# skyepurchase/MeatModeler

Hardware: AMD Instinct MI355X
Metric: descriptor-match pairs/sec + BA residuals/sec, 500×1080p frames, 1/2/4/8 GPU (higher is better)
Workload: dtype u8/int32 (match), f64 (BA); 1 GPU; 500 frames 1920x1080, 4000 ORB kpts/frame, BF Hamming 2-NN + ratio, track linking, 2-view DLT, full BA (TRF, Schur, f64 MFMA Cholesky); frames=500, height=1080, width=1920, nfeatures=4000, parallelism=pairs/points x1

## Files before the change

### meatmodeler_amd/csrc/ba.hip

```cpp
#include "ba_eval.h"


namespace {

template <bool FIXED>
__device__ __forceinline__ const double *cam_at(const double *__restrict__ cams, const double *__restrict__ fxc, int F, int f) {
    if constexpr (FIXED)
        return f < F ? cams + (size_t)f * 6 : fxc + (size_t)(f - F) * 6;
    else
        return cams + (size_t)f * 6;
}

template <bool FIXED>
__device__ __forceinline__ void ba_residual_body(mm_ba_problem pb, const double *__restrict__ cams, const double *__restrict__ fxc,
                                                          const double *__restrict__ pts, const CamCoef *__restrict__ ctab, double *__restrict__ res,
                                                          double *__restrict__ partial, const unsigned bx, const unsigned gx) {
    __shared__ double sm[4];
    __shared__ double Ks[9];
    if (threadIdx.x < 9) Ks[threadIdx.x] = pb.K[threadIdx.x];
    __syncthreads();
    double acc = 0;
    for (int64_t o = (int64_t)bx * 256 + threadIdx.x; o < pb.O; o += (int64_t)gx * 256) {
        Proj pr;
        const int f = pb.fi[o];
// ... 46 lines not shown
}
__global__ __launch_bounds__(256) void sum_partials_publish_kernel(const double *__restrict__ partial, int n,
                                                                   double *__restrict__ board, int cost_slot, int count,
                                                                   MMHostBoard *hb, unsigned long long seq) { sum_partials_publish_body(partial, n, board, cost_slot, count, hb, seq, blockIdx.x, gridDim.x); }

__global__ __launch_bounds__(256) void ba_jacobian_kernel(mm_ba_problem pb, const double *__restrict__ cams,
                                                          const double *__restrict__ pts, const CamCoef *__restrict__ ctab, double *__restrict__ Jc,
                                                          double *__restrict__ Jp) {
    __shared__ double Ks[9];
    if (threadIdx.x < 9) Ks[threadIdx.x] = pb.K[threadIdx.x];
    __syncthreads();
    int64_t o = (int64_t)blockIdx.x * 256 + threadIdx.x;
    if (o >= pb.O) return;
    Proj pr;
    const int f = pb.fi[o];
    ba_eval_cc<true, true>(cams + (size_t)f * 6, ctab[f],
                           pts + (size_t)pb.pi[o] * 3, Ks, pb.obs[2 * o], pb.obs[2 * o + 1], pr);
#pragma unroll
    for (int k = 0; k < 6; ++k) {
        Jc[o * 12 + k] = pr.Jc[0][k];
        Jc[o * 12 + 6 + k] = pr.Jc[1][k];
    }
#pragma unroll
    for (int k = 0; k < 3; ++k) {
        Jp[o * 6 + k] = pr.Jp[0][k];
        Jp[o * 6 + 3 + k] = pr.Jp[1][k];
    }
}

#ifndef MM_PB_LANES
#define MM_PB_LANES 4
#endif
constexpr int PB_LANES = MM_PB_LANES;
template <bool FIXED>
__device__ __forceinline__ void ba_point_blocks_body(mm_ba_problem pb, const double *__restrict__ cams, const double *__restrict__ fxc,
                                                              const double *__restrict__ pts, const CamCoef *__restrict__ ctab, double *__restrict__ C,
                                                              double *__restrict__ gp, const unsigned bx, const unsigned gx) {
    __shared__ double Ks[9];
    if (threadIdx.x < 9) Ks[threadIdx.x] = pb.K[threadIdx.x];
    __syncthreads();
    const int sub = threadIdx.x & (PB_LANES - 1);
    const int p = bx * (256 / PB_LANES) + (threadIdx.x / PB_LANES);
    const bool live = p < pb.P;
    double c[9] = {0, 0, 0, 0, 0, 0, 0, 0, 0};
    if (live) {
        const double *Xp = pts + (size_t)p * 3;
        const int e_end = pb.pt_ptr[p + 1];
        for (int e = pb.pt_ptr[p] + sub; e < e_end; e += PB_LANES) {
            const int o = pb.pt_obs[e];
            Proj pr;
            const int f = pb.fi[o];
            ba_eval_cc<false, true>(cam_at<FIXED>(cams, fxc, pb.F, f), ctab[f], Xp, Ks, pb.obs[2 * (size_t)o], pb.obs[2 * (size_t)o + 1], pr);
#pragma unroll
            for (int m = 0; m < 2; ++m) {
                const double j0 = pr.Jp[m][0], j1 = pr.Jp[m][1], j2 = pr.Jp[m][2];
                const double r = m == 0 ? pr.r0 : pr.r1;
                c[0] += j0 * j0; c[1] += j0 * j1; c[2] += j0 * j2;
                c[3] += j1 * j1; c[4] += j1 * j2; c[5] += j2 * j2;
                c[6] += j0 * r; c[7] += j1 * r; c[8] += j2 * r;
            }
        }
    }
#pragma unroll
    for (int off = 1; off < PB_LANES; off <<= 1) {
        double t[9];
#pragma unroll
        for (int q = 0; q < 9; ++q) t[q] = __shfl_xor(c[q], off, 64);
#pragma unroll
        for (int q = 0; q < 9; ++q) c[q] += t[q];
    }
    if (live && sub == 0) {
        double *Cp = C + (size_t)p * 6;
#pragma unroll
        for (int q = 0; q < 6; ++q) Cp[q] = c[q];
        gp[(size_t)p * 3] = c[6]; gp[(size_t)p * 3 + 1] = c[7]; gp[(size_t)p * 3 + 2] = c[8];
    }
}
__global__ __launch_bounds__(256) void ba_point_blocks_kernel(mm_ba_problem pb, const double *__restrict__ cams,
                                                              const double *__restrict__ pts, const CamCoef *__restrict__ ctab, double *__restrict__ C,
                                                              double *__restrict__ gp) { ba_point_blocks_body<false>(pb, cams, nullptr, pts, ctab, C, gp, blockIdx.x, gridDim.x); }
__global__ __launch_bounds__(256) void ba_point_blocks_fixed_kernel(mm_ba_problem pb, const double *__restrict__ cams, const double *__restrict__ fxc,
                                                                    const double *__restrict__ pts, const CamCoef *__restrict__ ctab, double *__restrict__ C,
// ... 29 lines not shown
            acc[21 + i] += pr.Jc[0][i] * pr.r0 + pr.Jc[1][i] * pr.r1;
        }
    }
    block_sum_n<27, 256>(acc, smn);
    if (threadIdx.x == 0) {
        int t = 0;
#pragma unroll
        for (int i = 0; i < 6; ++i) {
#pragma unroll
            for (int j = i; j < 6; ++j) {
                B[(size_t)f * 36 + i * 6 + j] = acc[t];
                B[(size_t)f * 36 + j * 6 + i] = acc[t];
                ++t;
            }
            gc[(size_t)f * 6 + i] = acc[21 + i];
        }
    }
}
__global__ __launch_bounds__(256) void ba_camera_blocks_kernel(mm_ba_problem pb, const double *__restrict__ cams,
                                                               const double *__restrict__ pts, double *__restrict__ B,
                                                               double *__restrict__ gc) { ba_camera_blocks_body(pb, cams, pts, B, gc, blockIdx.x, gridDim.x); }

__global__ __launch_bounds__(256) void ba_normal_eq_kernel(mm_ba_problem pb, const double *__restrict__ cams, const double *__restrict__ pts,
                                                           const CamCoef *__restrict__ ctab, double *__restrict__ B, double *__restrict__ gc,
                                                           double *__restrict__ C, double *__restrict__ gp) {
    if ((int)blockIdx.x < pb.F) ba_camera_blocks_body(pb, cams, pts, B, gc, blockIdx.x, (unsigned)pb.F);
    else ba_point_blocks_body<false>(pb, cams, nullptr, pts, ctab, C, gp, blockIdx.x - (unsigned)pb.F, gridDim.x - (unsigned)pb.F);
}
__global__ __launch_bounds__(256) void ba_normal_eq_fixed_kernel(mm_ba_problem pb, const double *__restrict__ cams, const double *__restrict__ fxc,
                                                                 const double *__restrict__ pts, const CamCoef *__restrict__ ctab, double *__restrict__ B,
                                                                 double *__restrict__ gc, double *__restrict__ C, double *__restrict__ gp) {
    if ((int)blockIdx.x < pb.F) ba_camera_blocks_body(pb, cams, pts, B, gc, blockIdx.x, (unsigned)pb.F);
    else ba_point_blocks_body<true>(pb, cams, fxc, pts, ctab, C, gp, blockIdx.x - (unsigned)pb.F, gridDim.x - (unsigned)pb.F);
}

__global__ __launch_bounds__(256) void ba_jvp_kernel(mm_ba_problem pb, const double *__restrict__ cams,
                                                     const double *__restrict__ pts, const CamCoef *__restrict__ ctab, const double *__restrict__ wc,
                                                     const double *__restrict__ wp, double *__restrict__ out) {
    __shared__ double Ks[9];
    if (threadIdx.x < 9) Ks[threadIdx.x] = pb.K[threadIdx.x];
    __syncthreads();
    int64_t o = (int64_t)blockIdx.x * 256 + threadIdx.x;
    if (o >= pb.O) return;
    const int f = pb.fi[o], p = pb.pi[o];
    Proj pr;
    ba_eval_cc<true, true>(cams + (size_t)f * 6, ctab[f],
                           pts + (size_t)p * 3, Ks, pb.obs[2 * o], pb.obs[2 * o + 1], pr);
    double y0 = 0, y1 = 0;
    if (wc) {
#pragma unroll
        for (int k = 0; k < 6; ++k) {
            double w = wc[(size_t)f * 6 + k];
            y0 += pr.Jc[0][k] * w;
            y1 += pr.Jc[1][k] * w;
        }
    }
    if (wp) {
#pragma unroll
        for (int k = 0; k < 3; ++k) {
            double w = wp[(size_t)p * 3 + k];
            y0 += pr.Jp[0][k] * w;
            y1 += pr.Jp[1][k] * w;
        }
    }
    out[2 * o] = y0;
    out[2 * o + 1] = y1;
// ... 127 lines not shown
                                                                double *__restrict__ dp, const unsigned bx, const unsigned gx) {
    const int sub = threadIdx.x & (PB_LANES - 1);
    const int p = bx * (256 / PB_LANES) + (threadIdx.x / PB_LANES);
    const bool live = p < pb.P;
    double t[3] = {0.0, 0.0, 0.0};
    if (live) {
        const int e_end = pb.pt_ptr[p + 1];
        for (int e = pb.pt_ptr[p] + sub; e < e_end; e += PB_LANES) {
            t[0] += T[3 * (size_t)e];
            t[1] += T[3 * (size_t)e + 1];
            t[2] += T[3 * (size_t)e + 2];
        }
    }
#pragma unroll
    for (int off = 1; off < PB_LANES; off <<= 1) {
        double u[3];
#pragma unroll
        for (int q = 0; q < 3; ++q) u[q] = __shfl_xor(t[q], off, 64);
#pragma unroll
        for (int q = 0; q < 3; ++q) t[q] += u[q];
    }
    if (live && sub == 0) {
        const double t0 = gp[(size_t)p * 3] - t[0], t1 = gp[(size_t)p * 3 + 1] - t[1], t2 = gp[(size_t)p * 3 + 2] - t[2];
        const double *c = Cinv + (size_t)p * 6;
        dp[(size_t)p * 3] = c[0] * t0 + c[1] * t1 + c[2] * t2;
        dp[(size_t)p * 3 + 1] = c[1] * t0 + c[3] * t1 + c[4] * t2;
        dp[(size_t)p * 3 + 2] = c[2] * t0 + c[4] * t1 + c[5] * t2;
    }
}
__global__ __launch_bounds__(256) void ba_backsub_points_kernel(mm_ba_problem pb, const double *__restrict__ T,
                                                                const double *__restrict__ Cinv, const double *__restrict__ gp,
                                                                double *__restrict__ dp) { ba_backsub_points_body(pb, T, Cinv, gp, dp, blockIdx.x, gridDim.x); }

__device__ __forceinline__ void cam_coef_body(const double *__restrict__ cams, int F, CamCoef *__restrict__ tab, const unsigned bx, const unsigned gx) {
    const int f = bx * 256 + threadIdx.x;
    if (f < F) tab[f] = cam_coef_of(cams + (size_t)f * 6);
}
__global__ __launch_bounds__(256) void cam_coef_kernel(const double *__restrict__ cams, int F, CamCoef *__restrict__ tab) { cam_coef_body(cams, F, tab, blockIdx.x, gridDim.x); }

int check_pb(mm_ctx *ctx, const mm_ba_problem *pb, const char *who) {
    if (!ctx) return MM_ERR_ARG;
    if (!pb || pb->F < 0 || pb->P < 0 || pb->O < 0 || !pb->K) return mm_fail(ctx, MM_ERR_ARG, "%s: bad problem", who);
    if (pb->O > 0 && (!pb->fi || !pb->pi || !pb->obs)) return mm_fail(ctx, MM_ERR_ARG, "%s: null observation arrays", who);
    return MM_OK;
}

constexpr int RES_BLOCKS = 2048;
constexpr int JVP_MAX_WG = 2048;
inline int res_wg_cap() {
    static const int cap = [] {
        const char *e = getenv("MM_RES_WG");
        const int v = e ? atoi(e) : RES_BLOCKS;
        return v < 1 ? 1 : (v > RES_BLOCKS ? RES_BLOCKS : v);
    }();
    return cap;
}
inline int jvp_wg_cap() {
    static const int cap = [] {
        const char *e = getenv("MM_JVP_WG");
        const int v = e ? atoi(e) : 1024;
        return v < 1 ? 1 : (v > JVP_MAX_WG ? JVP_MAX_WG : v);
    }();
    return cap;
}

__device__ __forceinline__ void trf_damping_body(const double *__restrict__ gh2, const double *__restrict__ d11, double Delta,
// ... 94 lines not shown
        ctx->cam_tab_for = cams;
        ctx->cam_tab_F = F;
    }
    if (ctx->fx_F > 0 && !ctx->fx_tab_ok) {
        MM_LAUNCH(ctx, "cam_coef_kernel", cam_coef_kernel, dim3((ctx->fx_F + 255) / 256), dim3(256), 0, ctx->fx_cams, ctx->fx_F,
                  (CamCoef *)ctx->cam_tab + F);
        ctx->fx_tab_ok = true;
    }
    *tab_out = ctx->cam_tab;
    return MM_OK;
}
int mm_cam_table_adopt(mm_ctx *ctx, const double *cams, int F, void **tab_out) {
    const int rows = F + ctx->fx_F;
    if (rows > ctx->cam_tab_cap) {
        if (ctx->cam_tab) (void)hipFree(ctx->cam_tab);
        ctx->cam_tab = nullptr;
        ctx->cam_tab_cap = 0;
        const int cap = rows < 1024 ? 1024 : rows + rows / 2;
        MM_HIP(ctx, hipMalloc(&ctx->cam_tab, (size_t)cap * sizeof(CamCoef)));
        ctx->cam_tab_cap = cap;
        ctx->fx_tab_ok = false;
    }
    ctx->cam_tab_for = cams;
    ctx->cam_tab_F = F;
    *tab_out = ctx->cam_tab;
    return MM_OK;
}
void mm_cam_table_hold(mm_ctx *ctx, bool on) {
    ctx->cam_tab_hold = on;
    ctx->cam_tab_for = nullptr;
}
void mm_cam_table_invalidate(mm_ctx *ctx) { ctx->cam_tab_for = nullptr; }

int mm_ba_residual_publish(mm_ctx *ctx, const mm_ba_problem *pb, const double *cams, const double *pts, void *ws,
                           size_t ws_bytes, double *board, int cost_slot, int count, void *host_board, unsigned long long seq);

#define MM_CAM_TABLE(ctx, pb, cams)                                               \
    const CamCoef *ctab = nullptr;                                                \
    do {                                                                          \
        const void *t_ = nullptr;                                                 \
        int rc_ = mm_cam_coef_table(ctx, cams, (pb)->F, &t_);                     \
        if (rc_) return rc_;                                                      \
        ctab = (const CamCoef *)t_;                                               \
    } while (0)

extern "C" {

int mm_ba_residual(mm_ctx *ctx, const mm_ba_problem *pb, const double *cams, const double *pts, double *res,
                   double *cost2, void *ws, size_t ws_bytes) {
    int rc = check_pb(ctx, pb, "mm_ba_residual");
    if (rc) return rc;
    if (!cams || !pts || !cost2) return mm_fail(ctx, MM_ERR_ARG, "mm_ba_residual: null pointer");
    if (!ws || ws_bytes < RES_BLOCKS * sizeof(double)) return mm_fail(ctx, MM_ERR_WORKSPACE, "mm_ba_residual: workspace < 16 KiB");
    int64_t nb = (pb->O + 255) / 256;
    int blocks = (int)(nb < 1 ? 1 : (nb > res_wg_cap() ? res_wg_cap() : nb));
    MM_CAM_TABLE(ctx, pb, cams);
    if (ctx->fx_F > 0)
        MM_LAUNCH(ctx, "ba_residual_fixed_kernel", ba_residual_fixed_kernel, dim3(blocks), dim3(256), 0, *pb, cams, ctx->fx_cams, pts, ctab, res,
                  (double *)ws);
    else
        MM_LAUNCH(ctx, "ba_residual_kernel", ba_residual_kernel, dim3(blocks), dim3(256), 0, *pb, cams, pts, ctab, res, (double *)ws);
    MM_LAUNCH(ctx, "sum_partials_kernel", sum_partials_kernel, dim3(1), dim3(256), 0, (const double *)ws, blocks, cost2);
    return MM_OK;
}

int mm_ba_jacobian(mm_ctx *ctx, const mm_ba_problem *pb, const double *cams, const double *pts, double *Jc, double *Jp) {
    int rc = check_pb(ctx, pb, "mm_ba_jacobian");
    if (rc) return rc;
    if (!cams || !pts || !Jc || !Jp) return mm_fail(ctx, MM_ERR_ARG, "mm_ba_jacobian: null pointer");
    if (ctx->fx_F > 0) return mm_fail(ctx, MM_ERR_ARG, "mm_ba_jacobian: no fixed-camera form");
    if (pb->O == 0) return MM_OK;
    MM_CAM_TABLE(ctx, pb, cams);
    MM_LAUNCH(ctx, "ba_jacobian_kernel", ba_jacobian_kernel, dim3((unsigned)((pb->O + 255) / 256)), dim3(256), 0, *pb, cams, pts, ctab, Jc, Jp);
    return MM_OK;
}

int mm_ba_normal_eq(mm_ctx *ctx, const mm_ba_problem *pb, const double *cams, const double *pts, double *B, double *gc,
                    double *C, double *gp) {
    int rc = check_pb(ctx, pb, "mm_ba_normal_eq");
    if (rc) return rc;
    if (!cams || !pts) return mm_fail(ctx, MM_ERR_ARG, "mm_ba_normal_eq: null pointer");
    if ((B == nullptr) != (gc == nullptr) || (C == nullptr) != (gp == nullptr))
        return mm_fail(ctx, MM_ERR_ARG, "mm_ba_normal_eq: B/gc and C/gp come in pairs");
    if (B && C && pb->P > 0 && pb->F > 0) {
        if (!pb->pt_ptr || !pb->pt_obs || !pb->cam_ptr || !pb->cam_obs) return mm_fail(ctx, MM_ERR_ARG, "mm_ba_normal_eq: CSR missing");
        MM_CAM_TABLE(ctx, pb, cams);
        const unsigned g_pblk = (unsigned)((pb->P + 256 / PB_LANES - 1) / (256 / PB_LANES));
        if (ctx->fx_F > 0)
            MM_LAUNCH(ctx, "ba_normal_eq_fixed_kernel", ba_normal_eq_fixed_kernel, dim3((unsigned)pb->F + g_pblk), dim3(256), 0, *pb, cams,
                      ctx->fx_cams, pts, ctab, B, gc, C, gp);
        else
            MM_LAUNCH(ctx, "ba_normal_eq_kernel", ba_normal_eq_kernel, dim3((unsigned)pb->F + g_pblk), dim3(256), 0, *pb, cams, pts, ctab, B, gc, C, gp);
        return MM_OK;
    }
    if (C) {
        if (!pb->pt_ptr || !pb->pt_obs) return mm_fail(ctx, MM_ERR_ARG, "mm_ba_normal_eq: point CSR missing");
        if (pb->P > 0) {
            MM_CAM_TABLE(ctx, pb, cams);
            if (ctx->fx_F > 0)
                MM_LAUNCH(ctx, "ba_point_blocks_fixed_kernel", ba_point_blocks_fixed_kernel, dim3((pb->P + 256 / PB_LANES - 1) / (256 / PB_LANES)),
                          dim3(256), 0, *pb, cams, ctx->fx_cams, pts, ctab, C, gp);
            else
                MM_LAUNCH(ctx, "ba_point_blocks_kernel", ba_point_blocks_kernel, dim3((pb->P + 256 / PB_LANES - 1) / (256 / PB_LANES)), dim3(256), 0,
                          *pb, cams, pts, ctab, C, gp);
        }
    }
    if (B) {
        if (!pb->cam_ptr || !pb->cam_obs) return mm_fail(ctx, MM_ERR_ARG, "mm_ba_normal_eq: camera CSR missing");
        if (pb->F > 0) {
            MM_LAUNCH(ctx, "ba_camera_blocks_kernel", ba_camera_blocks_kernel, dim3(pb->F), dim3(256), 0, *pb, cams, pts, B, gc);
        }
    }
    return MM_OK;
}

int mm_ba_jvp(mm_ctx *ctx, const mm_ba_problem *pb, const double *cams, const double *pts, const double *wc,
              const double *wp, double *out) {
    int rc = check_pb(ctx, pb, "mm_ba_jvp");
    if (rc) return rc;
    if (!cams || !pts || !out) return mm_fail(ctx, MM_ERR_ARG, "mm_ba_jvp: null pointer");
    if (ctx->fx_F > 0) return mm_fail(ctx, MM_ERR_ARG, "mm_ba_jvp: no fixed-camera form");
// ... 22 lines not shown
    const int64_t n_all = (pb->O + 255) / 256;
    const unsigned n_wg = (unsigned)(n_all < jvp_wg_cap() ? n_all : jvp_wg_cap());
    MM_CAM_TABLE(ctx, pb, cams);
    if (ctx->fx_F > 0)
        MM_LAUNCH(ctx, "ba_jvp_fixed_kernel", ba_jvp_dots_fixed_kernel, dim3(n_wg), dim3(256), 0, *pb, cams, ctx->fx_cams, pts, ctab, wc, wp,
                  out, other, (double *)((char *)ws + 256));
    else
        MM_LAUNCH(ctx, "ba_jvp_kernel", ba_jvp_dots_kernel, dim3(n_wg), dim3(256), 0, *pb, cams, pts, ctab, wc, wp, out, other,
                  (double *)((char *)ws + 256));
    if (ctx->jvp_rows_deferred) {
        ctx->jvp_partial = (const double *)((char *)ws + 256);
        ctx->jvp_n_wg = n_wg;
        return MM_OK;
    }
    MM_LAUNCH(ctx, "jvp_rows_kernel", jvp_rows_kernel, dim3(1), dim3(256), 0, (const double *)((char *)ws + 256), n_wg, rows);
    return MM_OK;
}

size_t mm_ba_backsub_workspace_bytes(const mm_ba_problem *pb) {
    if (!pb || pb->O <= 0) return 256;
    return mm_align_up((size_t)pb->O * 3 * sizeof(double), 256);
}

int mm_ba_backsub(mm_ctx *ctx, const mm_ba_problem *pb, const double *cams, const double *pts, const double *Cinv,
                  const double *gp, const double *dc, double *dp, void *ws, size_t ws_bytes) {
    int rc = check_pb(ctx, pb, "mm_ba_backsub");
    if (rc) return rc;
    if (!cams || !pts || !Cinv || !gp || !dc || !dp || !pb->pt_ptr || !pb->pt_obs)
        return mm_fail(ctx, MM_ERR_ARG, "mm_ba_backsub: null pointer");
    if (ws && ws_bytes < mm_ba_backsub_workspace_bytes(pb)) return mm_fail(ctx, MM_ERR_WORKSPACE, "mm_ba_backsub: workspace too small");
    if (pb->P == 0) return MM_OK;
    if (ctx->fx_F > 0 && !ws) return mm_fail(ctx, MM_ERR_WORKSPACE, "mm_ba_backsub: fixed cameras need the workspace");
    MM_CAM_TABLE(ctx, pb, cams);
    if (ws && pb->O > 0) {
        if (ctx->fx_F > 0)
            MM_LAUNCH(ctx, "ba_backsub_fixed_kernel", ba_backsub_obs_fixed_kernel, dim3((unsigned)((pb->O + 255) / 256)), dim3(256), 0, *pb,
                      cams, ctx->fx_cams, pts, ctab, dc, (double *)ws);
        else
            MM_LAUNCH(ctx, "ba_backsub_kernel", ba_backsub_obs_kernel, dim3((unsigned)((pb->O + 255) / 256)), dim3(256), 0, *pb, cams, pts,
                      ctab, dc, (double *)ws);
        MM_LAUNCH(ctx, "ba_backsub_points_kernel", ba_backsub_points_kernel, dim3((pb->P + 256 / PB_LANES - 1) / (256 / PB_LANES)), dim3(256), 0,
                  *pb, (const double *)ws, Cinv, gp, dp);
        return MM_OK;
    }
    MM_LAUNCH(ctx, "ba_backsub_kernel", ba_backsub_kernel, dim3((pb->P + 255) / 256), dim3(256), 0, *pb, cams, pts, ctab, Cinv, gp, dc, dp);
    return MM_OK;
}

static int mm_ba_fixed_check(mm_ctx *ctx, const mm_ba_fixed *fx, const char *who) {
    if (fx->F_fixed < 0 || (fx->F_fixed > 0 && !fx->cams)) return mm_fail(ctx, MM_ERR_ARG, "%s: bad fixed-camera descriptor", who);
    return MM_OK;
}

int mm_ba_residual_fixed(mm_ctx *ctx, const mm_ba_problem *pb, const mm_ba_fixed *fx, const double *cams, const double *pts,
                         double *res, double *cost2, void *ws, size_t ws_bytes) {
    if (!ctx) return MM_ERR_ARG;
    if (!fx || fx->F_fixed == 0) return mm_ba_residual(ctx, pb, cams, pts, res, cost2, ws, ws_bytes);
    int rc = mm_ba_fixed_check(ctx, fx, "mm_ba_residual_fixed");
    if (rc) return rc;
    mm_fixed_scope scope(ctx, fx);
    return mm_ba_residual(ctx, pb, cams, pts, res, cost2, ws, ws_bytes);
}

int mm_ba_normal_eq_fixed(mm_ctx *ctx, const mm_ba_problem *pb, const mm_ba_fixed *fx, const double *cams, const double *pts,
                          double *B, double *gc, double *C, double *gp) {
    if (!ctx) return MM_ERR_ARG;
// ... 91 lines not shown
```

### meatmodeler_amd/csrc/mm_common.h

```cpp
#pragma once
#include <hip/hip_runtime.h>
#include <cstdarg>
#include <cstdio>
#include <cstring>
#include <vector>
#include "../../include/meatmodeler.h"

struct mm_prof_rec {
    const char *name;
    hipEvent_t a, b;
};

struct mm_ctx {
    int device;
    hipStream_t stream;
    char err[512];
    int prof = 0;
    char prof_only[64] = {0};
    std::vector<mm_prof_rec> recs;
    std::vector<hipEvent_t> pool;
    hipStream_t aux = nullptr;
    hipEvent_t ev_fork = nullptr, ev_join = nullptr;
    bool attr_chol_fused = false, attr_chol_bwd = false, attr_chol_batch = false;
    int cu_count = 0, fused_wgs = 0, chol_last_path = -1, debug_abandon = 0;
    bool chol_avoid_fused = false;
    bool chol_strict_budget = false;
    hipEvent_t fused_ev = nullptr;
    bool fused_ev_pending = false;
    bool fused_no_event = false;
    int link_last_variant = -1;
    void *cam_tab = nullptr;
    int cam_tab_cap = 0, cam_tab_F = 0;
    const double *cam_tab_for = nullptr;
    bool cam_tab_hold = false;
    const double *fx_cams = nullptr;
    int fx_F = 0;
    bool fx_tab_ok = false;
    void *host_board = nullptr;
    unsigned long long host_board_seq = 0;
    void *batch_dev = nullptr, *batch_host = nullptr;
    size_t batch_dev_cap = 0, batch_host_cap = 0;
    bool jvp_rows_deferred = false;
    const double *jvp_partial = nullptr;
    unsigned jvp_n_wg = 0;
    const void *chol_init_done = nullptr;
    int chol_init_sides = 0;
    int batch_last = -1;
};

struct mm_stream_swap {
    mm_ctx *c;
    hipStream_t saved;
    mm_stream_swap(mm_ctx *ctx, hipStream_t s) : c(ctx), saved(ctx->stream) { ctx->stream = s; }
    ~mm_stream_swap() { c->stream = saved; }
};

struct mm_fixed_scope {
    mm_ctx *c;
    mm_fixed_scope(mm_ctx *ctx, const mm_ba_fixed *fx) : c(ctx) {
        ctx->fx_cams = fx->cams;
        ctx->fx_F = fx->F_fixed;
        ctx->fx_tab_ok = false;
    }
    ~mm_fixed_scope() {
        c->fx_cams = nullptr;
        c->fx_F = 0;
        c->fx_tab_ok = false;
    }
};

int mm_cam_coef_table(mm_ctx *ctx, const double *cams, int F, const void **tab_out);
void mm_cam_table_hold(mm_ctx *ctx, bool on);
void mm_cam_table_invalidate(mm_ctx *ctx);

int mm_ba_residual_publish(mm_ctx *ctx, const mm_ba_problem *pb, const double *cams, const double *pts, void *ws,
                           size_t ws_bytes, double *board, int cost_slot, int count, void *host_board, unsigned long long seq);

int mm_trf_fused0_scaled(mm_ctx *ctx, const double *g, double *si, const double *B, const double *C, double *gh, double *ghs, int64_t n,
                         int64_t split, double *out, void *ws, size_t ws_bytes);
int mm_trf_fused5_coef(mm_ctx *ctx, const double *x, const double *s1, const double *s2, double *x_new, const double *h01, int64_t n,
                       int64_t split, void *ctab, int F);
int mm_trf_rows_step2d(mm_ctx *ctx, const double *partial, unsigned n_wg, double *rows, const double *r0, const double *d11,
                       const double *r1, const double *r2, const double *r3, const double *reg, const int32_t *info, double Delta,
                       double *board);
int mm_cam_table_adopt(mm_ctx *ctx, const double *cams, int F, void **tab_out);
int mm_ba_damp_damping(mm_ctx *ctx, int F, int P, const double *B, const double *C, const double *scale_inv, const double *gh2,
                       const double *d11, double Delta, double min_damping, double *damp_out, double *Bd, double *Cd);
void mm_chol_release_budget(mm_ctx *ctx);
bool mm_chol_fused_eligible(int n, int half_bandwidth);
struct mm_chol_geom {
    int n, nblk, bwb;
    int a, m, b;
    int pad;
};
struct mm_chol_layout {
    double *Linv, *ytmp, *contrib, *contrib_bwd, *lpub, *spub;
    int32_t *flags;
    mm_chol_geom g;
    uint64_t nflags, nsent, nlpub;
};
struct mm_chol_plan {
    mm_chol_layout lay;
    bool fused;
    int sides;
    unsigned grid_fused, grid_bwd;
};
// ... 132 lines not shown
```

### meatmodeler_amd/csrc/trf.hip

```cpp
#include "mm_common.h"
#include "trf_decide.h"
#include <chrono>
#include <vector>
#include <algorithm>
#include <initializer_list>
#include <utility>
#include <cmath>
#include <cstdlib>

namespace {

__global__ __launch_bounds__(256) void vec_mul_kernel(const double *__restrict__ a, const double *__restrict__ b,
                                                      double *__restrict__ out, int64_t n) {
    const int64_t i = (int64_t)blockIdx.x * 256 + threadIdx.x;
    if (i < n) out[i] = a[i] * b[i];
}

struct HostBoard {
    double v[16];
    unsigned long long seq;
    unsigned long long pad[7];
};

__global__ __launch_bounds__(64) void board_publish_kernel(const double *__restrict__ dev, int count, HostBoard *hb,
// ... 73 lines not shown
    if (row / 6 == j / 6) v -= dup * Bd[(j / 6) * 36 + (row % 6) * 6 + j % 6];
    S[row * n + j] = v;
}
__global__ __launch_bounds__(256) void dedup_dense_kernel(double *__restrict__ S, int64_t n, const double *__restrict__ Bd, double dup) {
    const int64_t i = (int64_t)blockIdx.x * 256 + threadIdx.x;
    if (i >= n * 6) return;
    const int64_t f = i / 36, a = (i % 36) / 6, b = i % 6;
    S[(6 * f + a) * n + 6 * f + b] -= dup * Bd[i];
}
__global__ __launch_bounds__(256) void axpy_kernel(double *__restrict__ y, const double *__restrict__ x, double a, int64_t n) {
    const int64_t i = (int64_t)blockIdx.x * 256 + threadIdx.x;
    if (i < n) y[i] += a * x[i];
}

struct Carve {
    char *p;
    size_t used = 0;
    explicit Carve(void *base) : p((char *)base) {}
    template <class T>
    T *take(size_t count) {
        T *r = p ? (T *)(p + used) : nullptr;
        used += mm_align_up(count * sizeof(T), 256);
        return r;
    }
};

struct TrfWs {
    double *x, *x_new, *g, *si, *gh, *ghs, *gn, *q1, *w, *q2, *s1, *s2;
    double *B, *Bd, *C, *Cd, *Cinv, *u1, *Jq2, *dp, *v, *S;
    double *r0, *r1, *r2, *r3, *d11, *bs, *damp, *board, *cost2, *rowsx;
    int32_t *info;
    void *ws_res, *ws_md, *ws_jvp, *ws_schur, *ws_chol, *ws_back;
    size_t ws_res_b, ws_md_b, ws_jvp_b, ws_schur_b, ws_chol_b, ws_back_b;
    double *exs, *ex;
    size_t ex_count;
    size_t total;
};

TrfWs carve_trf(const mm_ba_problem *pb, void *base, int64_t ex_half_bw = -1) {
    TrfWs t;
    Carve c(base);
    const size_t F = pb->F, P = pb->P, O = (size_t)pb->O, n = 6 * F + 3 * P, nc = 6 * F;
    double **vecs[12] = {&t.x, &t.x_new, &t.g, &t.si, &t.gh, &t.ghs, &t.gn, &t.q1, &t.w, &t.q2, &t.s1, &t.s2};
    for (auto v : vecs) *v = c.take<double>(n + 2);
    t.B = c.take<double>(F * 36);
    t.Bd = c.take<double>(F * 36);
    t.C = c.take<double>(P * 6 + 2);
    t.Cd = c.take<double>(P * 6 + 2);
    t.Cinv = c.take<double>(P * 6 + 2);
    t.u1 = c.take<double>(O * 2 + 2);
    t.Jq2 = c.take<double>(O * 2 + 2);
    t.dp = c.take<double>(P * 3 + 2);
    t.v = c.take<double>(nc + 2);
    t.S = c.take<double>(2 * nc * nc + 2);
    t.r0 = c.take<double>(6);
    t.r1 = c.take<double>(9);
    t.r2 = c.take<double>(6);
    t.r3 = c.take<double>(18);
    t.d11 = c.take<double>(6);
    t.bs = c.take<double>(6);
    t.damp = c.take<double>(2);
    t.board = c.take<double>(16);
    t.cost2 = c.take<double>(1);
    t.rowsx = c.take<double>(3);
    t.info = c.take<int32_t>(1);
    t.ws_res_b = 2048 * 8;
    t.ws_res = c.take<char>(t.ws_res_b);
    t.ws_md_b = mm_multi_dot_workspace_bytes();
    t.ws_md = c.take<char>(t.ws_md_b);
    t.ws_jvp_b = mm_ba_jvp_dots_workspace_bytes(pb);
    t.ws_jvp = c.take<char>(t.ws_jvp_b);
    t.ws_schur_b = mm_ba_schur_workspace_bytes(pb);
    if (t.ws_schur_b < 256) t.ws_schur_b = 256;
    t.ws_schur = c.take<char>(t.ws_schur_b);
    t.ws_chol_b = mm_chol_workspace_bytes((int)nc);
    t.ws_chol = c.take<char>(t.ws_chol_b);
    t.ws_back_b = mm_ba_backsub_workspace_bytes(pb);
    t.ws_back = c.take<char>(t.ws_back_b);
    t.exs = nullptr;
    t.ex = nullptr;
    t.ex_count = 0;
    if (ex_half_bw >= 0) {
        const size_t hb = (size_t)(ex_half_bw < (int64_t)nc - 1 ? ex_half_bw : (nc ? nc - 1 : 0));
        t.ex_count = nc * (hb + 1) + nc;
        if (t.ex_count < F * 42) t.ex_count = F * 42;
        t.exs = c.take<double>(EX_SCALARS);
        t.ex = c.take<double>(t.ex_count + 2);
    }
    t.total = c.used;
    return t;
}

int wait_seq(mm_ctx *ctx, const unsigned long long *word, unsigned long long seq, const char *what, int problem = -1) {
    const auto t0 = std::chrono::steady_clock::now();
    unsigned long spins = 0;
    while (__atomic_load_n(word, __ATOMIC_ACQUIRE) != seq) {
        __builtin_ia32_pause();
        if ((++spins & 0xFFFFF) == 0 && std::chrono::steady_clock::now() - t0 > std::chrono::seconds(20)) {
            MM_HIP(ctx, hipStreamSynchronize(ctx->stream));
            if (__atomic_load_n(word, __ATOMIC_ACQUIRE) == seq) break;
            if (problem < 0) return mm_fail(ctx, MM_ERR_HIP, "%s never arrived", what);
            return mm_fail(ctx, MM_ERR_HIP, "%s %d never arrived", what, problem);
        }
    }
    return MM_OK;
}

using namespace mm_trf;

}

extern "C" size_t mm_ba_trf_workspace_bytes(const mm_ba_problem *pb) {
    if (!pb || pb->F < 0 || pb->P < 0 || pb->O < 0) return 0;
    return carve_trf(pb, nullptr).total;
}

#define TRF_CALL(expr)        \
    do {                      \
        int rc_ = (expr);     \
        if (rc_) return rc_;  \
    } while (0)

extern "C" size_t mm_ba_trf_dist_workspace_bytes(const mm_ba_problem *pb, int half_bandwidth) {
    if (!pb || pb->F < 0 || pb->P < 0 || pb->O < 0 || half_bandwidth < 0) return 0;
    return carve_trf(pb, nullptr, half_bandwidth).total;
}

static int trf_run(mm_ctx *ctx, const mm_ba_problem *pb, double *cams, double *pts, const mm_trf_params *prm, mm_trf_report *rep,
                   mm_trf_row *log, int log_cap, void *ws, size_t ws_bytes, const mm_dist *dist) {
    const auto t_enter = std::chrono::steady_clock::now();
    if (!ctx) return MM_ERR_ARG;
    if (!pb || !cams || !pts || !prm || !rep || pb->F <= 0 || pb->P < 0 || pb->O < 0 || !pb->K || log_cap < 0 || (log_cap > 0 && !log))
        return mm_fail(ctx, MM_ERR_ARG, "mm_ba_trf: bad argument");
    if (dist && (dist->world < 1 || dist->world > EX_MAX_WORLD || dist->rank < 0 || dist->rank >= dist->world || !dist->allreduce ||
                 dist->half_bandwidth < 0))
        return mm_fail(ctx, MM_ERR_ARG, "mm_ba_trf_dist: bad communicator description (1 <= world <= %d)", EX_MAX_WORLD);
    const size_t need = dist ? mm_ba_trf_dist_workspace_bytes(pb, dist->half_bandwidth) : mm_ba_trf_workspace_bytes(pb);
    if (!ws || ws_bytes < need || ((uintptr_t)ws & 255))
        return mm_fail(ctx, MM_ERR_WORKSPACE, "mm_ba_trf: workspace too small or misaligned");
    const TrfWs t = carve_trf(pb, ws, dist ? dist->half_bandwidth : -1);
    struct TableHold {
        mm_ctx *c;
        explicit TableHold(mm_ctx *ctx) : c(ctx) { mm_cam_table_hold(c, true); }
        ~TableHold() { mm_cam_table_hold(c, false); }
    } table_hold(ctx);
    struct FusedGuard {
        mm_ctx *c;
        bool saved, saved_strict, saved_no_event;
        FusedGuard(mm_ctx *ctx, bool sharded)
            : c(ctx), saved(ctx->chol_avoid_fused), saved_strict(ctx->chol_strict_budget), saved_no_event(ctx->fused_no_event) {
            c->fused_no_event = true;
            if (sharded) c->chol_strict_budget = true;
        }
        ~FusedGuard() {
            c->chol_avoid_fused = saved;
            c->chol_strict_budget = saved_strict;
            c->fused_no_event = saved_no_event;
            mm_chol_release_budget(c);
        }
    } fused_guard(ctx, dist != nullptr);
    const int F = pb->F, P = pb->P;
    const int64_t nc = 6 * (int64_t)F, n = nc + 3 * (int64_t)P;
    hipStream_t st = ctx->stream;
    auto pts_of = [&](double *v) { return v + nc; };
    MM_HIP(ctx, hipMemsetAsync(t.ws_md, 0, t.ws_md_b, st));
    MM_HIP(ctx, hipMemsetAsync(t.ws_jvp, 0, t.ws_jvp_b, st));
    MM_HIP(ctx, hipMemsetAsync(t.S, 0, (size_t)(2 * nc * nc) * sizeof(double), st));
    double *x = t.x, *x_new = t.x_new;
    MM_HIP(ctx, hipMemcpyAsync(x, cams, (size_t)nc * sizeof(double), hipMemcpyDeviceToDevice, st));
    if (P) MM_HIP(ctx, hipMemcpyAsync(x + nc, pts, (size_t)3 * P * sizeof(double), hipMemcpyDeviceToDevice, st));
    double host[16];
    rep->chol_fallbacks = 0;
    rep->collectives = 0;
// ... 17 lines not shown
        TRF_CALL(ar(t.exs, EX_SCALARS));
        hipLaunchKernelGGL(ex_unpack_kernel, dim3(1), dim3(64), 0, st, it, (const double *)t.exs);
        MM_LAUNCH_CHECK(ctx, "ex_unpack_kernel");
        return MM_OK;
    };
    auto normal_eq = [&](double *v) -> int {
        TRF_CALL(mm_ba_normal_eq(ctx, pb, v, pts_of(v), t.B, t.g, t.C, pts_of(t.g)));
        if (!dist) return MM_OK;
        MM_HIP(ctx, hipMemcpyAsync(t.ex, t.B, (size_t)F * 36 * sizeof(double), hipMemcpyDeviceToDevice, st));
        MM_HIP(ctx, hipMemcpyAsync(t.ex + (size_t)F * 36, t.g, (size_t)nc * sizeof(double), hipMemcpyDeviceToDevice, st));
        TRF_CALL(ar(t.ex, (int64_t)F * 42));
        MM_HIP(ctx, hipMemcpyAsync(t.B, t.ex, (size_t)F * 36 * sizeof(double), hipMemcpyDeviceToDevice, st));
        MM_HIP(ctx, hipMemcpyAsync(t.g, t.ex + (size_t)F * 36, (size_t)nc * sizeof(double), hipMemcpyDeviceToDevice, st));
        return MM_OK;
    };
    if (!ctx->host_board) {
        MM_HIP(ctx, hipHostMalloc(&ctx->host_board, sizeof(HostBoard), hipHostMallocDefault));
        memset(ctx->host_board, 0, sizeof(HostBoard));
        ctx->host_board_seq = 0;
    }
    HostBoard *hb = (HostBoard *)ctx->host_board;
    auto take_board = [&](unsigned long long seq, int count) -> int {
        TRF_CALL(wait_seq(ctx, &hb->seq, seq, "mm_ba_trf: the trial-step scalars"));
        for (int i = 0; i < count; ++i) host[i] = ((volatile double *)hb->v)[i];
        mm_chol_release_budget(ctx);
        return MM_OK;
    };
    auto read_board = [&](const double *dev, int count) -> int {
        const unsigned long long seq = ++ctx->host_board_seq;
        hipLaunchKernelGGL(board_publish_kernel, dim3(1), dim3(64), 0, st, dev, count, hb, seq);
        MM_LAUNCH_CHECK(ctx, "board_publish_kernel");
        return take_board(seq, count);
    };
    TRF_CALL(mm_ba_residual(ctx, pb, x, pts_of(x), nullptr, t.cost2, t.ws_res, t.ws_res_b));
    if (dist) {
        const double av = ctx->chol_avoid_fused ? 1.0 : 0.0;
        MM_HIP(ctx, hipMemcpyAsync(t.board + 15, &av, sizeof(double), hipMemcpyHostToDevice, st));
        MM_HIP(ctx, hipStreamSynchronize(st));
        TRF_CALL(exchange({{t.cost2, 3}, {t.board + 15, 3}}));
        TRF_CALL(read_board(t.board + 15, 1));
        if (host[0] > 0) ctx->chol_avoid_fused = true;
    }
    TRF_CALL(read_board(t.cost2, 1));
    const double cost0 = 0.5 * host[0];
    rep->cost0 = cost0;
    if (!std::isfinite(cost0)) {
        rep->status = -2;
        return mm_fail(ctx, MM_ERR_NUMERIC, "mm_ba_trf: residuals are not finite in the initial point");
    }
    const int half_bw = dist ? dist->half_bandwidth : 6 * pb->cam_span + 5;
    TRF_CALL(normal_eq(x));
    TRF_CALL(mm_ba_scale_update(ctx, F, P, t.B, t.C, t.si, 1));
    {
        hipLaunchKernelGGL(vec_mul_kernel, dim3((unsigned)((n + 255) / 256)), dim3(256), 0, st, (const double *)x, (const double *)t.si, t.w, n);
        const double *pa[1] = {t.w}, *pbv[1] = {t.w};
        TRF_CALL(mm_multi_dot(ctx, 1, pa, pbv, n, nc, t.rowsx, t.ws_md, t.ws_md_b));
        TRF_CALL(exchange({{t.rowsx, 0}}));
        TRF_CALL(read_board(t.rowsx, 3));
    }
    TrfDecide d(cost0, host[2], n, *prm, log, log_cap);
    Outcome next = d.begin();
    static const bool timing = getenv("MM_TRF_TIMING") && atoi(getenv("MM_TRF_TIMING")) > 0;
    const auto t_loop = std::chrono::steady_clock::now();
    auto t_iter = t_loop;
    if (timing) fprintf(stderr, "mm_ba_trf timing: prologue %.1f us\n", std::chrono::duration<double, std::micro>(t_loop - t_enter).count());
    for (;;) {
        if (timing && d.iteration > 0) {
            const auto now = std::chrono::steady_clock::now();
            fprintf(stderr, "mm_ba_trf timing: iteration %d %.1f us (nfev %d)\n", d.iteration - 1,
                    std::chrono::duration<double, std::micro>(now - t_iter).count(), d.nfev);
            t_iter = now;
        }
        if (!dist && d.iteration > 0) {
            TRF_CALL(mm_trf_fused0_scaled(ctx, t.g, t.si, t.B, t.C, t.gh, t.ghs, n, nc, t.r0, t.ws_md, t.ws_md_b));
        } else {
            const double *in[2] = {t.g, t.si};
            double *outv[2] = {t.gh, t.ghs};
// ... 407 lines not shown
```

Before: 9382 billion descriptor pairs/s (match stage).

## Pre-gather camera-ordered observation streams and fuse point back-substitution for BA sweeps

Before the TRF loop, observations are gathered into camera-ordered arrays of point indices and xy coordinates. The code also checks whether pt_obs is the identity permutation, so the point-block path can skip that indirection. The camera-block normal-equation kernel now reads contiguous streams, prefetches the next point, and computes camera coefficients once per block. A new fused back-substitution kernel computes per-observation rows into shared memory and reduces them per point, replacing the separate observation pass. This costs extra workspace (O ints plus 2·O doubles) and a one-time gather, and changes the workspace size calculation.

Result: no change. 9291 billion descriptor pairs/s (match stage) (-1.0%).

```diff
diff --git a/meatmodeler_amd/csrc/ba.hip b/meatmodeler_amd/csrc/ba.hip
--- a/meatmodeler_amd/csrc/ba.hip
+++ b/meatmodeler_amd/csrc/ba.hip
@@ -102,7 +102,7 @@
 #define MM_PB_LANES 4
 #endif
 constexpr int PB_LANES = MM_PB_LANES;
-template <bool FIXED>
+template <bool FIXED, bool IDENT = false>
 __device__ __forceinline__ void ba_point_blocks_body(mm_ba_problem pb, const double *__restrict__ cams, const double *__restrict__ fxc,
                                                               const double *__restrict__ pts, const CamCoef *__restrict__ ctab, double *__restrict__ C,
                                                               double *__restrict__ gp, const unsigned bx, const unsigned gx) {
@@ -117,7 +117,8 @@
         const double *Xp = pts + (size_t)p * 3;
         const int e_end = pb.pt_ptr[p + 1];
         for (int e = pb.pt_ptr[p] + sub; e < e_end; e += PB_LANES) {
-            const int o = pb.pt_obs[e];
+            int o = e;
+            if constexpr (!IDENT) o = pb.pt_obs[e];
             Proj pr;
             const int f = pb.fi[o];
             ba_eval_cc<false, true>(cam_at<FIXED>(cams, fxc, pb.F, f), ctab[f], Xp, Ks, pb.obs[2 * (size_t)o], pb.obs[2 * (size_t)o + 1], pr);
@@ -213,6 +214,93 @@
                                                                  double *__restrict__ gc, double *__restrict__ C, double *__restrict__ gp) {
     if ((int)blockIdx.x < pb.F) ba_camera_blocks_body(pb, cams, pts, B, gc, blockIdx.x, (unsigned)pb.F);
     else ba_point_blocks_body<true>(pb, cams, fxc, pts, ctab, C, gp, blockIdx.x - (unsigned)pb.F, gridDim.x - (unsigned)pb.F);
+}
+
+__device__ __forceinline__ void ba_camera_blocks_streams_body(mm_ba_problem pb, const double *__restrict__ cams,
+                                                               const double *__restrict__ pts, const int32_t *__restrict__ cam_pi,
+                                                               const double *__restrict__ cam_xy, double *__restrict__ B,
+                                                               double *__restrict__ gc, const unsigned bx, const unsigned gx) {
+    __shared__ double smn[4 * 27];
+    __shared__ double Ks[9];
+    __shared__ double cs[6];
+    const int f = bx;
+    if (threadIdx.x < 9) Ks[threadIdx.x] = pb.K[threadIdx.x];
+    if (threadIdx.x < 6) cs[threadIdx.x] = cams[(size_t)f * 6 + threadIdx.x];
+    __syncthreads();
+    const CamCoef ccf = cam_coef_of(cs);
+    double acc[27];
+#pragma unroll
+    for (int i = 0; i < 27; ++i) acc[i] = 0;
+    const int e_end = pb.cam_ptr[f + 1], e_last = e_end - 1;
+    int e = pb.cam_ptr[f] + threadIdx.x;
+    int p_next = 0;
+    double X[3] = {0, 0, 0};
+    if (e < e_end) {
+        const int p = cam_pi[e];
+        p_next = cam_pi[e + 256 < e_last ? e + 256 : e_last];
+#pragma unroll
+        for (int k = 0; k < 3; ++k) X[k] = pts[(size_t)p * 3 + k];
+    }
+    while (e < e_end) {
+        const double ox = cam_xy[2 * (size_t)e], oy = cam_xy[2 * (size_t)e + 1];
+        double Xn[3];
+#pragma unroll
+        for (int k = 0; k < 3; ++k) Xn[k] = pts[(size_t)p_next * 3 + k];
+        p_next = cam_pi[e + 512 < e_last ? e + 512 : e_last];
+        Proj pr;
+        ba_eval_cc<true, false>(cs, ccf, X, Ks, ox, oy, pr);
+        int t = 0;
+#pragma unroll
+        for (int i = 0; i < 6; ++i) {
+#pragma unroll
+            for (int j = i; j < 6; ++j) {
+                acc[t] += pr.Jc[0][i] * pr.Jc[0][j] + pr.Jc[1][i] * pr.Jc[1][j];
+                ++t;
+            }
+            acc[21 + i] += pr.Jc[0][i] * pr.r0 + pr.Jc[1][i] * pr.r1;
+        }
+#pragma unroll
+        for (int k = 0; k < 3; ++k) X[k] = Xn[k];
+        e += 256;
+    }
+    block_sum_n<27, 256>(acc, smn);
+    if (threadIdx.x == 0) {
+        int t = 0;
+#pragma unroll
+        for (int i = 0; i < 6; ++i) {
+#pragma unroll
+            for (int j = i; j < 6; ++j) {
+                B[(size_t)f * 36 + i * 6 + j] = acc[t];
+                B[(size_t)f * 36 + j * 6 + i] = acc[t];
+                ++t;
+            }
+            gc[(size_t)f * 6 + i] = acc[21 + i];
+        }
+    }
+}
+template <bool FIXED, bool STREAM, bool IDENT>
+__global__ __launch_bounds__(256, 3) void ba_normal_eq_streams_kernel(mm_ba_problem pb, const double *__restrict__ cams, const double *__restrict__ fxc,
+                                                                   const double *__restrict__ pts, const CamCoef *__restrict__ ctab,
+                                                                   const int32_t *__restrict__ cam_pi, const double *__restrict__ cam_xy,
+                                                                   double *__restrict__ B, double *__restrict__ gc, double *__restrict__ C,
+                                                                   double *__restrict__ gp) {
+    if ((int)blockIdx.x < pb.F) {
+        if constexpr (STREAM) ba_camera_blocks_streams_body(pb, cams, pts, cam_pi, cam_xy, B, gc, blockIdx.x, (unsigned)pb.F);
+        else ba_camera_blocks_body(pb, cams, pts, B, gc, blockIdx.x, (unsigned)pb.F);
+    } else ba_point_blocks_body<FIXED, IDENT>(pb, cams, fxc, pts, ctab, C, gp, blockIdx.x - (unsigned)pb.F, gridDim.x - (unsigned)pb.F);
+}
+
+__global__ __launch_bounds__(256) void ba_streams_gather_kernel(mm_ba_problem pb, int32_t *__restrict__ cam_pi, double *__restrict__ cam_xy) {
+    const int64_t e = (int64_t)blockIdx.x * 256 + threadIdx.x;
+    if (e >= pb.O || e >= (int64_t)pb.cam_ptr[pb.F]) return;
+    const int o = pb.cam_obs[e];
+    cam_pi[e] = pb.pi[o];
+    cam_xy[2 * e] = pb.obs[2 * (size_t)o];
+    cam_xy[2 * e + 1] = pb.obs[2 * (size_t)o + 1];
+}
+__global__ __launch_bounds__(256) void ba_streams_ident_kernel(mm_ba_problem pb, double *__restrict__ not_ident) {
+    const int64_t e = (int64_t)blockIdx.x * 256 + threadIdx.x;
+    if (e < pb.O && (int64_t)pb.pt_obs[e] != e) not_ident[0] = 1.0;
 }
 
 __global__ __launch_bounds__(256) void ba_jvp_kernel(mm_ba_problem pb, const double *__restrict__ cams,
@@ -406,6 +494,83 @@
                                                                 const double *__restrict__ Cinv, const double *__restrict__ gp,
                                                                 double *__restrict__ dp) { ba_backsub_points_body(pb, T, Cinv, gp, dp, blockIdx.x, gridDim.x); }
 
+template <bool FIXED>
+__device__ __forceinline__ void ba_backsub_row(const mm_ba_problem &pb, const double *__restrict__ cams, const double *__restrict__ fxc,
+                                               const double *__restrict__ pts, const CamCoef *__restrict__ ctab,
+                                               const double *__restrict__ dc, const double *Ks, const int o, double (&row)[3]) {
+    const int f = pb.fi[o], p = pb.pi[o];
+    Proj pr;
+    ba_eval_cc<true, true>(cam_at<FIXED>(cams, fxc, pb.F, f), ctab[f], pts + (size_t)p * 3, Ks, pb.obs[2 * (size_t)o],
+                           pb.obs[2 * (size_t)o + 1], pr);
+    double s0 = 0, s1 = 0;
+    if (!FIXED || f < pb.F) {
+#pragma unroll
+        for (int k = 0; k < 6; ++k) {
+            const double d = dc[(size_t)f * 6 + k];
+            s0 += pr.Jc[0][k] * d;
+            s1 += pr.Jc[1][k] * d;
+        }
+    }
+    row[0] = fma(pr.Jp[0][0], s0, pr.Jp[1][0] * s1);
+    row[1] = fma(pr.Jp[0][1], s0, pr.Jp[1][1] * s1);
+    row[2] = fma(pr.Jp[0][2], s0, pr.Jp[1][2] * s1);
+}
+template <bool FIXED>
+__global__ __launch_bounds__(256, 6) void ba_backsub_fused_kernel(mm_ba_problem pb, const double *__restrict__ cams, const double *__restrict__ fxc,
+                                                               const double *__restrict__ pts, const CamCoef *__restrict__ ctab,
+                                                               const double *__restrict__ Cinv, const double *__restrict__ gp,
+                                                               const double *__restrict__ dc, double *__restrict__ dp) {
+    __shared__ double Ks[9];
+    __shared__ double Ts[3][256];
+    if (threadIdx.x < 9) Ks[threadIdx.x] = pb.K[threadIdx.x];
+    const int sub = threadIdx.x & (PB_LANES - 1);
+    const int p0 = blockIdx.x * (256 / PB_LANES);
+    const int p = p0 + (threadIdx.x / PB_LANES);
+    const bool live = p < pb.P;
+    const int p1 = p0 + 256 / PB_LANES < pb.P ? p0 + 256 / PB_LANES : pb.P;
+    const int c_begin = pb.pt_ptr[p0];
+    int c_end = pb.pt_ptr[p1];
+    if ((int64_t)c_end > pb.O) c_end = (int)pb.O;
+    int e = live ? pb.pt_ptr[p] + sub : 0;
+    int e_end = live ? pb.pt_ptr[p + 1] : 0;
+    if (e_end > c_end) e_end = c_end;
+    double t[3] = {0.0, 0.0, 0.0};
+    __syncthreads();
+    for (int c0 = c_begin; c0 < c_end; c0 += 256) {
+        const int mine = c0 + (int)threadIdx.x;
+        if (mine < c_end) {
+            double row[3];
+            ba_backsub_row<FIXED>(pb, cams, fxc, pts, ctab, dc, Ks, mine, row);
+            Ts[0][threadIdx.x] = row[0];
+            Ts[1][threadIdx.x] = row[1];
+            Ts[2][threadIdx.x] = row[2];
+        }
+        __syncthreads();
+        const int stop = e_end < c0 + 256 ? e_end : c0 + 256;
+        for (; e < stop; e += PB_LANES) {
+            t[0] += Ts[0][e - c0];
+            t[1] += Ts[1][e - c0];
+            t[2] += Ts[2][e - c0];
+        }
+        __syncthreads();
+    }
+#pragma unroll
+    for (int off = 1; off < PB_LANES; off <<= 1) {
+        double u[3];
+#pragma unroll
+        for (int q = 0; q < 3; ++q) u[q] = __shfl_xor(t[q], off, 64);
+#pragma unroll
+        for (int q = 0; q < 3; ++q) t[q] += u[q];
+    }
+    if (live && sub == 0) {
+        const double t0 = gp[(size_t)p * 3] - t[0], t1 = gp[(size_t)p * 3 + 1] - t[1], t2 = gp[(size_t)p * 3 + 2] - t[2];
+        const double *c = Cinv + (size_t)p * 6;
+        dp[(size_t)p * 3] = c[0] * t0 + c[1] * t1 + c[2] * t2;
+        dp[(size_t)p * 3 + 1] = c[1] * t0 + c[3] * t1 + c[4] * t2;
+        dp[(size_t)p * 3 + 2] = c[2] * t0 + c[4] * t1 + c[5] * t2;
+    }
+}
+
 __device__ __forceinline__ void cam_coef_body(const double *__restrict__ cams, int F, CamCoef *__restrict__ tab, const unsigned bx, const unsigned gx) {
     const int f = bx * 256 + threadIdx.x;
     if (f < F) tab[f] = cam_coef_of(cams + (size_t)f * 6);
@@ -566,8 +731,40 @@
 }
 void mm_cam_table_invalidate(mm_ctx *ctx) { ctx->cam_tab_for = nullptr; }
 
+int mm_sweep_streams_parts(const mm_ba_problem *pb) {
+    if (pb->O <= 0 || pb->P <= 0 || pb->F <= 0 || !pb->pi || !pb->obs || !pb->pt_ptr || !pb->pt_obs || !pb->cam_ptr || !pb->cam_obs) return 0;
+    const char *e = getenv("MM_BA_STREAMS");
+    return e ? atoi(e) & MM_SS_ALL : MM_SS_ALL;
+}
+int mm_sweep_streams_fill(mm_ctx *ctx, const mm_ba_problem *pb, int32_t *cam_pi, double *cam_xy, double *not_ident) {
+    const unsigned g = (unsigned)((pb->O + 255) / 256);
+    MM_HIP(ctx, hipMemsetAsync(not_ident, 0, sizeof(double), ctx->stream));
+    MM_LAUNCH(ctx, "ba_streams_gather_kernel", ba_streams_gather_kernel, dim3(g), dim3(256), 0, *pb, cam_pi, cam_xy);
+    MM_LAUNCH(ctx, "ba_streams_ident_kernel", ba_streams_ident_kernel, dim3(g), dim3(256), 0, *pb, not_ident);
+    return MM_OK;
+}
+static int sweep_streams_for(const mm_ctx *ctx, const mm_ba_problem *pb) {
+    if (!ctx->ss_parts || ctx->ss_for != pb->cam_obs || ctx->ss_O != pb->O) return 0;
+    return ctx->ss_ident ? ctx->ss_parts : ctx->ss_parts & MM_SS_CAMERA;
+}
+
 int mm_ba_residual_publish(mm_ctx *ctx, const mm_ba_problem *pb, const double *cams, const double *pts, void *ws,
                            size_t ws_bytes, double *board, int cost_slot, int count, void *host_board, unsigned long long seq);
+
+template <bool FIXED>
+static int normal_eq_streams(mm_ctx *ctx, const char *name, int ss, dim3 grid, const mm_ba_problem *pb, const double *cams, const double *pts,
+                             const CamCoef *ctab, double *B, double *gc, double *C, double *gp) {
+    if (ss == (MM_SS_CAMERA | MM_SS_POINT))
+        MM_LAUNCH(ctx, name, (ba_normal_eq_streams_kernel<FIXED, true, true>), grid, dim3(256), 0, *pb, cams, ctx->fx_cams, pts, ctab,
+                  ctx->ss_cam_pi, ctx->ss_cam_xy, B, gc, C, gp);
+    else if (ss == MM_SS_CAMERA)
+        MM_LAUNCH(ctx, name, (ba_normal_eq_streams_kernel<FIXED, true, false>), grid, dim3(256), 0, *pb, cams, ctx->fx_cams, pts, ctab,
+                  ctx->ss_cam_pi, ctx->ss_cam_xy, B, gc, C, gp);
+    else
+        MM_LAUNCH(ctx, name, (ba_normal_eq_streams_kernel<FIXED, false, true>), grid, dim3(256), 0, *pb, cams, ctx->fx_cams, pts, ctab,
+                  ctx->ss_cam_pi, ctx->ss_cam_xy, B, gc, C, gp);
+    return MM_OK;
+}
 
 #define MM_CAM_TABLE(ctx, pb, cams)                                               \
     const CamCoef *ctab = nullptr;                                                \
@@ -620,7 +817,12 @@
         if (!pb->pt_ptr || !pb->pt_obs || !pb->cam_ptr || !pb->cam_obs) return mm_fail(ctx, MM_ERR_ARG, "mm_ba_normal_eq: CSR missing");
         MM_CAM_TABLE(ctx, pb, cams);
         const unsigned g_pblk = (unsigned)((pb->P + 256 / PB_LANES - 1) / (256 / PB_LANES));
-        if (ctx->fx_F > 0)
+        const int ss = sweep_streams_for(ctx, pb) & (MM_SS_CAMERA | MM_SS_POINT);
+        if (ss) {
+            const dim3 grid((unsigned)pb->F + g_pblk);
+            return ctx->fx_F > 0 ? normal_eq_streams<true>(ctx, "ba_normal_eq_fixed_kernel", ss, grid, pb, cams, pts, ctab, B, gc, C, gp)
+                                 : normal_eq_streams<false>(ctx, "ba_normal_eq_kernel", ss, grid, pb, cams, pts, ctab, B, gc, C, gp);
+        } else if (ctx->fx_F > 0)
             MM_LAUNCH(ctx, "ba_normal_eq_fixed_kernel", ba_normal_eq_fixed_kernel, dim3((unsigned)pb->F + g_pblk), dim3(256), 0, *pb, cams,
                       ctx->fx_cams, pts, ctab, B, gc, C, gp);
         else
@@ -709,6 +911,16 @@
     if (pb->P == 0) return MM_OK;
     if (ctx->fx_F > 0 && !ws) return mm_fail(ctx, MM_ERR_WORKSPACE, "mm_ba_backsub: fixed cameras need the workspace");
     MM_CAM_TABLE(ctx, pb, cams);
+    if (ws && (sweep_streams_for(ctx, pb) & MM_SS_BACKSUB)) {
+        const dim3 grid((unsigned)((pb->P + 256 / PB_LANES - 1) / (256 / PB_LANES)));
+        if (ctx->fx_F > 0)
+            MM_LAUNCH(ctx, "ba_backsub_fixed_kernel", ba_backsub_fused_kernel<true>, grid, dim3(256), 0, *pb, cams, ctx->fx_cams, pts, ctab,
+                      Cinv, gp, dc, dp);
+        else
+            MM_LAUNCH(ctx, "ba_backsub_kernel", ba_backsub_fused_kernel<false>, grid, dim3(256), 0, *pb, cams, (const double *)nullptr, pts,
+                      ctab, Cinv, gp, dc, dp);
+        return MM_OK;
+    }
     if (ws && pb->O > 0) {
         if (ctx->fx_F > 0)
             MM_LAUNCH(ctx, "ba_backsub_fixed_kernel", ba_backsub_obs_fixed_kernel, dim3((unsigned)((pb->O + 255) / 256)), dim3(256), 0, *pb,
diff --git a/meatmodeler_amd/csrc/mm_common.h b/meatmodeler_amd/csrc/mm_common.h
--- a/meatmodeler_amd/csrc/mm_common.h
+++ b/meatmodeler_amd/csrc/mm_common.h
@@ -46,6 +46,28 @@
     const void *chol_init_done = nullptr;
     int chol_init_sides = 0;
     int batch_last = -1;
+    const int32_t *ss_cam_pi = nullptr;
+    const double *ss_cam_xy = nullptr;
+    const int32_t *ss_for = nullptr;
+    int64_t ss_O = 0;
+    int ss_parts = 0;
+    bool ss_ident = false;
+};
+
+enum { MM_SS_CAMERA = 1, MM_SS_POINT = 2, MM_SS_BACKSUB = 4, MM_SS_ALL = 7 };
+
+struct mm_sweep_scope {
+    mm_ctx *c;
+    explicit mm_sweep_scope(mm_ctx *ctx) : c(ctx) { close(); }
+    ~mm_sweep_scope() { close(); }
+    void close() {
+        c->ss_cam_pi = nullptr;
+        c->ss_cam_xy = nullptr;
+        c->ss_for = nullptr;
+        c->ss_O = 0;
+        c->ss_parts = 0;
+        c->ss_ident = false;
+    }
 };
 
 struct mm_stream_swap {
@@ -72,6 +94,9 @@
 int mm_cam_coef_table(mm_ctx *ctx, const double *cams, int F, const void **tab_out);
 void mm_cam_table_hold(mm_ctx *ctx, bool on);
 void mm_cam_table_invalidate(mm_ctx *ctx);
+
+int mm_sweep_streams_parts(const mm_ba_problem *pb);
+int mm_sweep_streams_fill(mm_ctx *ctx, const mm_ba_problem *pb, int32_t *cam_pi, double *cam_xy, double *not_ident);
 
 int mm_ba_residual_publish(mm_ctx *ctx, const mm_ba_problem *pb, const double *cams, const double *pts, void *ws,
                            size_t ws_bytes, double *board, int cost_slot, int count, void *host_board, unsigned long long seq);
diff --git a/meatmodeler_amd/csrc/trf.hip b/meatmodeler_amd/csrc/trf.hip
--- a/meatmodeler_amd/csrc/trf.hip
+++ b/meatmodeler_amd/csrc/trf.hip
@@ -129,6 +129,8 @@
     int32_t *info;
     void *ws_res, *ws_md, *ws_jvp, *ws_schur, *ws_chol, *ws_back;
     size_t ws_res_b, ws_md_b, ws_jvp_b, ws_schur_b, ws_chol_b, ws_back_b;
+    int32_t *cam_pi;
+    double *cam_xy;
     double *exs, *ex;
     size_t ex_count;
     size_t total;
@@ -158,7 +160,7 @@
     t.bs = c.take<double>(6);
     t.damp = c.take<double>(2);
     t.board = c.take<double>(16);
-    t.cost2 = c.take<double>(1);
+    t.cost2 = c.take<double>(2);
     t.rowsx = c.take<double>(3);
     t.info = c.take<int32_t>(1);
     t.ws_res_b = 2048 * 8;
@@ -174,6 +176,8 @@
     t.ws_chol = c.take<char>(t.ws_chol_b);
     t.ws_back_b = mm_ba_backsub_workspace_bytes(pb);
     t.ws_back = c.take<char>(t.ws_back_b);
+    t.cam_pi = c.take<int32_t>(O);
+    t.cam_xy = c.take<double>(2 * O);
     t.exs = nullptr;
     t.ex = nullptr;
     t.ex_count = 0;
@@ -234,8 +238,10 @@
         return mm_fail(ctx, MM_ERR_ARG, "mm_ba_trf_dist: bad communicator description (1 <= world <= %d)", EX_MAX_WORLD);
     const size_t need = dist ? mm_ba_trf_dist_workspace_bytes(pb, dist->half_bandwidth) : mm_ba_trf_workspace_bytes(pb);
     if (!ws || ws_bytes < need || ((uintptr_t)ws & 255))
-        return mm_fail(ctx, MM_ERR_WORKSPACE, "mm_ba_trf: workspace too small or misaligned");
+        return mm_fail(ctx, MM_ERR_WORKSPACE, "mm_ba_trf: workspace too small (%zu bytes, needs %zu) or misaligned", ws ? ws_bytes : (size_t)0, need);
     const TrfWs t = carve_trf(pb, ws, dist ? dist->half_bandwidth : -1);
+    mm_sweep_scope sweep_scope(ctx);
+    const int ss_parts = mm_sweep_streams_parts(pb);
     struct TableHold {
         mm_ctx *c;
         explicit TableHold(mm_ctx *ctx) : c(ctx) { mm_cam_table_hold(c, true); }
@@ -319,6 +325,7 @@
         MM_LAUNCH_CHECK(ctx, "board_publish_kernel");
         return take_board(seq, count);
     };
+    if (ss_parts) TRF_CALL(mm_sweep_streams_fill(ctx, pb, t.cam_pi, t.cam_xy, t.cost2 + 1));
     TRF_CALL(mm_ba_residual(ctx, pb, x, pts_of(x), nullptr, t.cost2, t.ws_res, t.ws_res_b));
     if (dist) {
         const double av = ctx->chol_avoid_fused ? 1.0 : 0.0;
@@ -328,8 +335,16 @@
         TRF_CALL(read_board(t.board + 15, 1));
         if (host[0] > 0) ctx->chol_avoid_fused = true;
     }
-    TRF_CALL(read_board(t.cost2, 1));
+    TRF_CALL(read_board(t.cost2, ss_parts ? 2 : 1));
     const double cost0 = 0.5 * host[0];
+    if (ss_parts) {
+        ctx->ss_cam_pi = t.cam_pi;
+        ctx->ss_cam_xy = t.cam_xy;
+        ctx->ss_for = pb->cam_obs;
+        ctx->ss_O = pb->O;
+        ctx->ss_ident = host[1] == 0.0;
+        ctx->ss_parts = ss_parts;
+    }
     rep->cost0 = cost0;
     if (!std::isfinite(cost0)) {
         rep->status = -2;
```
